# oss0430/SRFRD

Hardware: AMD Instinct MI355X
Metric: sequences/sec (higher is better)
Workload: dtype f32

## Files before the change

srfrd_amd/csrc/srfrd_encoder_bwd_ragged_kernel.inc:

```
namespace SRFRD_NS {


struct RagBwdLds {
  lds_f* base;
  lds_f* s_ln;
  lds_f* s_lng;
};

template <int K_, int DI_, bool RMW_, bool SEAM_ = false>
__device__ __forceinline__ void rag_bwd_seq(const EncArgs& a, const RagBwdLds& m, int b, int iter, int& tid, int wave, uint32_t seed,
                                            int seam_th = 0) {
  const Dims& ly = a.dm;
  constexpr int nw = 8, nthr = 512;
  constexpr int L = 50, D = 50, LP = 64, DK = 52, DS = 54, NT = 4, MT = 4;
  constexpr int R = 52, SZ = R * DS, SLD = R + 2, SH = kRagSH;
  static_assert(SH == LP - R && R * SLD <= SZ + 2 * R, "slot geometry");
  static_assert(kRagBwdWork == SH * DS + 6 * SZ + 13 * LP, "working set");
  constexpr bool CV2 = true;
  constexpr int CIT = (R * (D / 2) + nthr - 1) / nthr;
  constexpr int PIT = (R * (R / 2) + nthr - 1) / nthr;
  lds_f* slot[6];
#pragma unroll
  for (int s = 0; s < 6; ++s) slot[s] = m.base + SH * DS + s * SZ;
  lds_f* tail = m.base + SH * DS + 6 * SZ;
  lds_i* s_in = (lds_i*)tail;
  lds_f* s_keep = tail + LP;
  lds_i* s_pid = (lds_i*)(tail + 2 * LP);
  lds_i* s_nid = (lds_i*)(tail + 3 * LP);
  lds_i* s_fk = (lds_i*)(tail + 4 * LP);
  lds_i* s_pfk = (lds_i*)(tail + 5 * LP);
  lds_i* s_nfk = (lds_i*)(tail + 6 * LP);
  lds_f* s_dpl = tail + 7 * LP;
  lds_f* s_dnl = tail + 8 * LP;
  lds_f* s_delta = tail + 9 * LP;
  lds_f* s_brep = tail + 10 * LP;
  lds_f* s_dummy = tail + 11 * LP;
  lds_f* s_misc = tail + 12 * LP;
  lds_f* s_ln = m.s_ln;
  lds_f* s_lng = m.s_lng;
  const float* P = a.dense;
  const bool drop_on = a.drop_on != 0;
  const int rkind = K_ >= 0 ? K_ : ly.kind;
  const bool is_sas = rkind == SRFRD_SASREC;
  const bool has_fake = rkind == SRFRD_SRFR || rkind == SRFRD_SRFRN;
  const bool is_srfu = rkind >= SRFRD_SRFU_B;
  constexpr int di = DI_, dfk = D - DI_;
  constexpr int dout = (K_ == SRFRD_SRFR) ? DI_ : D;
  const float sqrtD = sqrtf((float)di);
  const float qscale = a.qscale;
  const int B = a.B;
  auto pk = [&](int mat, int form) {
    return PackedB{reinterpret_cast<const float4*>(a.packed) + ((int64_t)mat * 2 + form) * (kPackFloats / 4)};
  };
  static_assert(L <= nthr && (R - L) * DS <= nthr, "single-pass helpers");
  auto ones_col = [&](lds_f* buf) {
    if (tid < L) buf[tid * DS + D] = 1.0f;
  };
  auto zero_pad_rows = [&](lds_f* buf) {
    if (tid < (R - L) * DS) buf[L * DS + tid] = 0.f;
  };
  const float keep_scale = drop_on ? a.drop_scale : 1.0f;

  asm volatile("" : "+v"(tid));
  float* slab = a.grad_slabs + (int64_t)blockIdx.x * ly.n_dense;
  const int rmw = RMW_ ? (iter != 0) : 0;
  if (iter == 0)
    for (int i = tid; i < ly.blk0; i += nthr) slab[i] = 0.f;
  const int64_t rowbase = (int64_t)b * L;
  const uint32_t seq = (uint32_t)(a.seq0 + b);
  const int lane0 = tid & 63;
  if (tid < LP) {
    const int t = tid;
    const bool in = t < L;
    const int id = in ? clamp_id(a.in_ids[rowbase + t], ly.n_items) : 0;
    const int pid = (in && a.pos_ids) ? clamp_id(a.pos_ids[rowbase + t], ly.n_items) : 0;
    const int nid = (in && a.neg_ids) ? clamp_id(a.neg_ids[rowbase + t], ly.n_items) : 0;
    s_in[t] = id;
    s_keep[t] = id != 0 ? 1.f : 0.f;
    s_pid[t] = pid;
    s_nid[t] = nid;
    s_fk[t] = (in && a.fk_ids) ? clamp_id(a.fk_ids[rowbase + t], 2) : 0;
    s_pfk[t] = (in && a.pos_fk) ? clamp_id(a.pos_fk[rowbase + t], 2) : 0;
    s_nfk[t] = (in && a.neg_fk) ? clamp_id(a.neg_fk[rowbase + t], 2) : 0;
    float dp = 0.f, dn = 0.f;
    if constexpr (SEAM_) {
      if constexpr (K_ == SRFRD_SRFRN)
        if (in) {
          const float* dl = a.head_dh + (int64_t)B * L * dout + rowbase * 2;
          dp = dl[t];
          dn = dl[L + t];
        }
    } else if (in) {
      if (a.fused_bce) {
        const float pl = a.c_pl[rowbase + t], nl = a.c_nl[rowbase + t];
        bce_dlogits(pid, pl, nl, dp, dn);
      } else {
        if (a.d_pos && a.pos_ids) dp = a.d_pos[rowbase + t];
        if (a.d_neg && a.neg_ids) dn = a.d_neg[rowbase + t];
      }
    }
    s_dpl[t] = dp;
    s_dnl[t] = dn;
  }
  if (is_srfu && wave == 1) {
    const int lab = user_label_wave(rkind, a.fk_ids ? a.fk_ids + rowbase : nullptr, L, ly.n_labels);
    if (lane0 == 0) ((lds_i*)s_misc)[0] = lab;
  }
  __syncthreads();
  int t0, th;
  {
    const bool inr = lane0 < L;
    const unsigned long long nz = __ballot(inr && s_in[lane0] != 0);
    const unsigned long long ng = __ballot(inr && (s_in[lane0] != 0 || s_dpl[lane0] != 0.f || s_dnl[lane0] != 0.f));
    t0 = nz ? (int)__builtin_ctzll(nz) : L;
    th = ng ? (int)__builtin_ctzll(ng) : L;
    if (a.ragged_off) t0 = 0;
    if (a.d_hidden != nullptr || a.ragged_off) th = 0;
    if constexpr (SEAM_) th = seam_th;
    t0 = __builtin_amdgcn_readfirstlane(t0);
    th = __builtin_amdgcn_readfirstlane(th);
  }
  const int krp = t0 >= 1 ? t0 - 1 : 0;
  const int kr = krp + SH, v0 = t0 + SH;
  const int mt0 = kr >> 4, r0 = mt0 << 4, mtn = MT - mt0;
  const int p0 = r0 > SH ? r0 - SH : 0;
  const int k0 = p0 + SH;
  const RagHead hr = rag_head_range(th, krp);
  const int mh0 = hr.tile0, mhn = MT - mh0;
  const int ph0 = hr.pos0, kh0 = ph0 + SH;

  lds_f *sX = slot[0], *sQ = slot[1], *sG = slot[2], *sT = slot[3], *sK = slot[4], *sO = slot[5];
  lds_f* dummy = s_dummy;
#define TB(p) ((p) - SH * DS)
  G2L<CIT, CV2> g_last, g_h1, g_r;
  g_last.load(a.c_save_x + x_off(ly.n_blocks, b, ly.n_blocks, L, D) + p0 * D, L - p0, D, nthr);
  g_h1.load(a.c_save_h1 + h1_off(ly.n_blocks - 1, b, ly.n_blocks, L, D) + p0 * D, L - p0, D, nthr);
  g_r.load(a.c_save_aux + aux_off(ly.n_blocks - 1, b, ly.n_blocks, L, LP, D).r + p0 * D, L - p0, D, nthr);
  if constexpr (SEAM_) {
    constexpr bool V2 = dout % 2 == 0;
    constexpr int HIT = (L * (V2 ? dout / 2 : dout) + nthr - 1) / nthr;
    G2L<HIT, V2> g_dh;
    g_dh.load(a.head_dh + (rowbase + ph0) * dout, L - ph0, dout, nthr);
    g_dh.store(sG + ph0 * DS, DS, L - ph0, dout, nthr);
    if constexpr (K_ == SRFRD_SRFRN) {
      g_dh.load(a.c_hidden + (rowbase + ph0) * dout, L - ph0, dout, nthr);
      g_dh.store(sT + ph0 * DS, DS, L - ph0, dout, nthr);
    }
    if (dout < D)
      for (int idx = tid; idx < (L - ph0) * (D - dout); idx += nthr) {
        const int tt = idx / (D - dout), cc = dout + idx - tt * (D - dout);
        sG[(ph0 + tt) * DS + cc] = 0.f;
      }
  }
  g_last.store(sX + p0 * DS, DS, L - p0, D, nthr);
  for (int r = ph0 + (tid >> 6); r < p0; r += nthr >> 6) {
    const int c = tid & 63;
    if (c < DS && c != D) sX[r * DS + c] = 0.f;
  }
  zero_pad_rows(sX);
  ones_col(sX);
  zero_pad_rows(sG);
  __syncthreads();

  int lane = tid & 63, li = lane & 15, lq = lane >> 4;
#define RG_RELANE() do { asm volatile("" : "+v"(tid)); lane = tid & 63; li = lane & 15; lq = lane >> 4; } while (0)
  const int nt_w = wave & 3, g_w = wave >> 2;
  auto slab_gemm = [&](int kk0, auto amat, auto bmat, const SlabWB& sl, const SlabPre& pre) {
    f32x4 acc[2];
#pragma unroll
    for (int j = 0; j < 2; ++j) acc[j] = f32x4{pre.v[j][0], pre.v[j][1], pre.v[j][2], pre.v[j][3]};
    mma_group<2>(acc, amat, bmat, (g_w << 4) + li, 32, (nt_w << 4) + li, kk0, LP, lq);
    const SlabCol sc = slab_col(sl, (nt_w << 4) + li);
    if (sc.ok) {
#pragma unroll
      for (int j = 0; j < 2; ++j)
#pragma unroll
        for (int e = 0; e < 4; ++e) {
          const int r = ((g_w + 2 * j) << 4) + (lq << 2) + e;
          if (r < sl.R) sl.base[(unsigned)(sc.col0 + r * sc.rs)] = acc[j][e];
        }
    }
  };
  auto col_sums = [&](int kk0, const lds_f* m_b, lds_f* dst, int ncol) {
    if (wave < NT) {
      f32x4 acc[1] = {f32x4{0.f, 0.f, 0.f, 0.f}};
      mma_group<1>(acc, OnesRow{}, Mat{m_b, DS}, li, 0, (wave << 4) + li, kk0, LP, lq);
      const int c = (wave << 4) + li;
      if (lq == 0 && c < ncol) dst[c] += acc[0][0];
    }
  };
  auto side_sums = [&](int n_out, auto term, auto dst_off, int tlo) {
    for (int p = wave; p < n_out; p += nw) {
      float sacc = 0.f;
      for (int t = tlo + lane; t < L; t += 64) sacc += term(p, t);
      sacc = wave_sum(sacc);
      if (lane == 0) atomicAdd(&slab[dst_off(p)], sacc);
    }
  };

  const lds_f* lnin = sX;
  if (K_ == SRFRD_SRFR) {
    const WFrag wl = load_wfrag(pk(ly.n_blocks * 6, 0), P + ly.off_lc_b, di, (di + 15) >> 4, tid);
    {
      constexpr int nst = (di + 15) >> 4;
      const int nt3 = wave % nst, g3 = wave / nst;
      auto epi = [&](int r, int c, float v) { *((c < di && r >= SH && r < SH + L) ? &TB(sQ)[r * DS + c] : dummy + c) = v; };
      if (g3 < 2) {
        if (g3 + 2 < mhn) gemm_group_packed<2>(mh0 + g3, 2, nt3, DK >> 2, Mat{TB(sX), DS}, wl, epi, lane);
        else if (g3 < mhn) gemm_group_packed<1>(mh0 + g3, 2, nt3, DK >> 2, Mat{TB(sX), DS}, wl, epi, lane);
      }
    }
    __syncthreads();
    lnin = sQ;
  }
  if constexpr (!SEAM_) {
// ... 345 lines not shown
    col_sums(k0, TB(H), s_lng + (4 * i + 1) * 64, D);
    col_sums(k0, TB(GX1), s_lng + (4 * i + 0) * 64, D);
    __syncthreads();
    G = DX;
    fr[0] = H; fr[1] = GX1; fr[2] = Xb; fr[3] = N1; fr[4] = DQ;
  }

  RG_RELANE();
  {
    const DropSite dsE = drop_site(drop_on && is_sas, seed, SITE_EMB, seq, a.drop_thr, a.drop_scale);
    {
      int t = p0 + tid / di, c = tid - (tid / di) * di;
      constexpr int dt = nthr / di, dc = nthr - dt * di;
      for (; t < L;) {
        float gv = G[t * DS + c] * s_keep[t];
        if (is_sas) gv *= drop_mul(dsE, t, c);
        const int id = s_in[t];
        if (a.contrib != nullptr) a.contrib[(((int64_t)2 * B + b) * L + t) * di + c] = id != 0 ? (is_sas ? gv * sqrtD : gv) : 0.f;
        else if (id != 0) atomicAdd(&a.grad_table[(int64_t)id * di + c], is_sas ? gv * sqrtD : gv);
        atomicAdd(&slab[ly.off_pos + t * di + c], gv);
        t += dt; c += dc;
        if (c >= di) { c -= di; ++t; }
      }
      if (a.contrib != nullptr)
        for (int idx = tid; idx < p0 * di; idx += nthr) a.contrib[(((int64_t)2 * B + b) * L) * di + idx] = 0.f;
    }
    if (has_fake)
      side_sums(2 * dfk, [&](int p, int t) {
        constexpr int dq = dfk > 0 ? dfk : 1;
        const int f = 1 + p / dq, c = p - (f - 1) * dq;
        return s_fk[t] == f ? G[t * DS + di + c] * s_keep[t] : 0.f;
      }, [&](int p) { return ly.off_side + dfk + p; }, p0);
    if (is_srfu) {
      const int lab = ((lds_i*)s_misc)[0];
      side_sums(D, [&](int c, int t) { return G[t * DS + c] * s_keep[t]; }, [&](int c) { return ly.off_side + lab * D + c; }, p0);
    }
  }
  __syncthreads();
  for (int idx = tid; idx < (4 * ly.n_blocks + 2) * 64; idx += nthr) {
    const int vec = idx >> 6, c = idx & 63;
    if (vec < 4 * ly.n_blocks) {
      const BlkOff o = blk_off(ly.blk0 + (vec >> 2) * ly.blk_stride, D);
      const int sel = vec & 3;
      if (c < D) slab[(sel == 0 ? o.ln1_w : sel == 1 ? o.ln1_b : sel == 2 ? o.ln2_w : o.ln2_b) + c] = s_lng[idx];
    } else if (c < dout) {
      slab[(vec == 4 * ly.n_blocks ? ly.off_ll_w : ly.off_ll_b) + c] = s_lng[idx];
    }
  }
  __syncthreads();
#undef TB
#undef RG_RELANE
}

template <int K_, int DI_, bool RMW_>
__global__ void __launch_bounds__(512, 4) encoder_bwd_ragged_kernel(const EncArgs a) {
  extern __shared__ __attribute__((aligned(16))) float smem[];
  const Dims& ly = a.dm;
  constexpr int nthr = 512;
  int tid = threadIdx.x;
  const int wave = __builtin_amdgcn_readfirstlane(tid >> 6);
  const RagT0 t0v = rag_load_t0(a, tid);
  lds_f* base = (lds_f*)smem;
  {
    const int total = (int)bwd_ragged_lds_floats(ly.n_blocks);
    for (int i = tid; i < total; i += nthr) base[i] = 0.f;
  }
  lds_f* s_ln = base + kRagBwdWork;
  const RagBwdLds m{base, s_ln, s_ln + ln_cache_floats(ly.n_blocks)};
  __syncthreads();
  fill_ln_cache(s_ln, a.dense, ly);
  const uint32_t seed = a.seed_dev ? *a.seed_dev : a.seed;
  __syncthreads();

  STAMP_INIT
  for (int iter = 0;; ++iter) {
    const int b = __builtin_amdgcn_readfirstlane(rag_take(a, (lds_i*)(base + kRagSH * 54), iter, tid, t0v));
    if (b < 0) break;
    rag_bwd_seq<K_, DI_, RMW_>(a, m, b, iter, tid, wave, seed);
  }
}

}
```

srfrd_amd/csrc/srfrd_encoder_fwd_ragged_kernel.inc:

```
namespace SRFRD_NS {

constexpr int kRagSH = 12;

constexpr int kRagChunks = 2;
struct RagT0 {
  int v[kRagChunks];
};
__device__ __forceinline__ bool rag_ordered(const EncArgs& a) { return a.sched != nullptr && a.sched_mode != 0 && a.B <= 512 * kRagChunks; }
__device__ __forceinline__ RagT0 rag_load_t0(const EncArgs& a, int tid) {
  RagT0 t;
#pragma unroll
  for (int c = 0; c < kRagChunks; ++c) {
    const int b = c * 512 + tid;
    t.v[c] = (rag_ordered(a) && c * 512 < a.B) ? a.sched[kSchedT0 + min(b, a.B - 1)] : 0;
  }
  return t;
}

__device__ __forceinline__ int rag_select(const RagT0& t0v, int B, int want, lds_i* scr, int tid) {
  lds_i* hist = scr;
  lds_i* wcnt = scr + 64;
  lds_i* res = scr + 80;
  const int lane = tid & 63, wave = tid >> 6;
  constexpr int NCH = kRagChunks;
// ... 25 lines not shown
  int seen = 0;
#pragma unroll
  for (int c = 0; c < NCH; ++c) {
    if (c * 512 >= B) break;
    const int b = c * 512 + tid;
    const bool f = b < B && min(max(tv[c], 0), 63) == k;
    const unsigned long long m = __ballot(f);
    if (lane == 0) wcnt[wave] = (int)__builtin_popcountll(m);
    __syncthreads();
    int before = seen, total = 0;
#pragma unroll
    for (int w = 0; w < 8; ++w) {
      const int cw = wcnt[w];
      if (w < wave) before += cw;
      total += cw;
    }
    const int mine = before + (int)__builtin_popcountll(m & ((1ull << lane) - 1ull));
    if (f && mine == r) res[2] = b;
    seen += total;
    __syncthreads();
  }
  return res[2];
}

__device__ __forceinline__ int rag_take(const EncArgs& a, lds_i* scr, int iter, int tid, const RagT0& t0v) {
  const int x = (int)blockIdx.x + iter * (int)gridDim.x;
  if (x >= a.B) return -1;
  if (!rag_ordered(a)) return x;
  const int G = a.sched[kSchedG];
  const int want = x < G ? x : (x < 2 * G ? a.B - 1 - (x - G) : x - G);
  return rag_select(t0v, a.B, want, scr, tid);
}

__device__ __forceinline__ float softplus_fast(float z) { return fmaxf(z, 0.f) + __logf(1.0f + __expf(-fabsf(z))); }

__device__ __forceinline__ void bce_dlogits(int pid, float pl, float nl, float& dp, float& dn) {
  if (pid != 0) {
    dp = sigmoid_f(pl) - 1.0f;
    dn = sigmoid_f(nl);
  }
}
__device__ __forceinline__ float head_dh(float up, float dp, float pv, float dn, float nv) {
  up += dp * pv + dn * nv;
  return up;
}
template <int K_>
__device__ __forceinline__ float head_dh_as_backward(float dp, float pv, float dn, float nv) {
  float a = dp * pv;
  asm volatile("" : "+v"(a));
  if constexpr (K_ == SRFRD_SRFRN) return __builtin_fmaf(dn, nv, a);
  float b = dn * nv;
  asm volatile("" : "+v"(b));
  return a + b;
}
__device__ __forceinline__ float head_contrib(float dl, float h) { return dl * h; }
struct RagHead {
  int tile0, pos0;
};
__device__ __forceinline__ RagHead rag_head_range(int th, int krp) {
  const int hp = th < krp ? th : krp;
  RagHead r;
  r.tile0 = (hp + kRagSH) >> 4;
  const int rh0 = r.tile0 << 4;
  r.pos0 = rh0 > kRagSH ? rh0 - kRagSH : 0;
  return r;
}

struct NoPost {
  __device__ __forceinline__ void operator()(int, int, const float (&)[4]) const {}
};
template <int G, bool TWO, class AL, class AL2, class PRE, class EPI, class POST = NoPost>
__device__ __forceinline__ void rgemm_packed(int mt, int mstride_tiles, int nt, int ksteps, int ncols, const AL& a, const WFrag& w,
                                             const AL2& a2, const WFrag& w2, const PRE& pre, const EPI& epi, int lane,
                                             const POST& post = POST{}) {
  const int li = lane & 15, lq = lane >> 4;
  const int c = (nt << 4) + li;
  float pv[G][4];
#pragma unroll
  for (int j = 0; j < G; ++j)
#pragma unroll
    for (int e = 0; e < 4; ++e) pv[j][e] = pre(((mt + j * mstride_tiles) << 4) + (lq << 2) + e, c);
  f32x4 acc[G];
#pragma unroll
  for (int j = 0; j < G; ++j) acc[j] = f32x4{0.f, 0.f, 0.f, 0.f};
  const int mrow = (mt << 4) + li, mstride = mstride_tiles << 4;
#pragma unroll
  for (int pass = 0; pass < (TWO ? 2 : 1); ++pass) {
    float av[4][G];
#pragma unroll
    for (int s = 0; s < 4; ++s)
      if (s < ksteps)
#pragma unroll
        for (int j = 0; j < G; ++j) av[s][j] = pass == 0 ? a(mrow + j * mstride, 4 * s + lq) : a2(mrow + j * mstride, 4 * s + lq);
#pragma unroll
    for (int kc = 0; kc < kPackKC; ++kc) {
      const int nst = ksteps - 4 * kc;
      if (nst > 0) {
        const int nnext = nst - 4;
        float an[4][G];
#pragma unroll
        for (int s = 0; s < 4; ++s)
          if (s < nnext)
#pragma unroll
            for (int j = 0; j < G; ++j)
              an[s][j] = pass == 0 ? a(mrow + j * mstride, ((kc + 1) << 4) + 4 * s + lq) : a2(mrow + j * mstride, ((kc + 1) << 4) + 4 * s + lq);
        __builtin_amdgcn_sched_barrier(0);
// ... 139 lines not shown
    for (int i = 0; i < 4; ++i) { const f32x2 t = row2[i < npair ? i : 0]; x[2 * i] = t.x; x[2 * i + 1] = t.y; }
  }
  float mx = -INFINITY;
#pragma unroll
  for (int i = 0; i < 8; ++i) {
    const int pj = m8 + i;
    x[i] = (own && pj >= krp && pj <= ip) ? x[i] : -INFINITY;
    mx = fmaxf(mx, x[i]);
  }
  mx = row_max(mx);
  float s = 0.f;
#pragma unroll
  for (int i = 0; i < 8; ++i) {
    const int pj = m8 + i;
    const float e = (own && pj >= krp && pj <= ip) ? __expf(x[i] - mx) : 0.f;
    x[i] = e;
    s += (rep && pj == krp) ? e * (float)t0 : e;
  }
  s = row_sum(s);
  const float inv = 1.0f / s;
  float cnt = (float)t0;
  if (ds.on && rep) {
    int c = 0;
    for (int jj = tid & 7; jj < t0; jj += 8) c += drop_mul(ds, ip, jj) != 0.f ? 1 : 0;
    cnt = row_sum((float)c);
  }
  if (!own) return;
  const float scale = ds.on ? ds.scale : 1.0f;
  float pv[8], gs[8];
#pragma unroll
  for (int i = 0; i < 8; ++i) {
    const int pj = m8 + i;
    const float p = x[i] * inv;
    if (rep && pj == krp) {
      const float pm = p * cnt;
      if (gsave != nullptr) gsave[ip * LP + LP - 1] = p * (float)t0;
      pv[i] = pm * scale;
      gs[i] = pm;
    } else {
      const float mul = drop_mul(ds, ip, pj);
      pv[i] = p * mul;
      gs[i] = mul != 0.f ? p : -p;
    }
  }
#pragma unroll
  for (int i = 0; i < 4; ++i)
    if (i < npair) row2[i] = f32x2{pv[2 * i], pv[2 * i + 1]};
  if (g4 != nullptr) {
    g4[0] = make_float4(gs[0], gs[1], gs[2], gs[3]);
    g4[1] = make_float4(gs[4], gs[5], gs[6], gs[7]);
  }
}

struct RagFwdLds {
  lds_f *bXS, *bQN, *bQ, *bK, *bV;
  lds_i* s_in;
  lds_f* s_keep;
  lds_i *s_pid, *s_nid;
  lds_f* s_misc;
  lds_f* s_ln;
};

template <int K_, int T_, int DI_, bool SEAM_ = false>
__device__ __forceinline__ int rag_fwd_seq(const EncArgs& a, const RagFwdLds& m, int b, int& tid, int wave, uint32_t seed) {
  static_assert(!SEAM_ || T_ != 0, "the head seam belongs to the training forward");
  const Dims& ly = a.dm;
  constexpr int D = 50, L = 50, LP = 64, DK = 52, DS = 54, SLD = 66, NT = 4, MT = 4, SH = kRagSH;
  constexpr int nw = 8, nthr = 512;
  static_assert(SH + L <= LP && (SH & 3) == 0, "tile coordinates");
  const int lane0 = threadIdx.x & 63;
  lds_f* bXS = m.bXS;
  lds_f* bQN = m.bQN;
  lds_f* bQ = m.bQ;
  lds_f* bK = m.bK;
  lds_f* bV = m.bV;
  lds_i* s_in = m.s_in;
  lds_f* s_keep = m.s_keep;
  lds_i* s_pid = m.s_pid;
  lds_i* s_nid = m.s_nid;
  lds_f* s_misc = m.s_misc;
  lds_f* s_ln = m.s_ln;
  const float* P = a.dense;
  const ItemTable table{a.table, a.table16};
  constexpr bool TR_ = T_ != 0;
  const bool has_pos = TR_ || a.pos_ids != nullptr, has_neg = TR_ || a.neg_ids != nullptr;
  const bool drop_on = TR_ || a.drop_on != 0, do_save = TR_ || a.save_x != nullptr, do_loss = TR_ || a.loss_part != nullptr;
  const int kind = K_ >= 0 ? K_ : ly.kind;
  const bool is_sas = kind == SRFRD_SASREC;
  const bool has_fake = kind == SRFRD_SRFR || kind == SRFRD_SRFRN;
  const bool is_srfu = kind >= SRFRD_SRFU_B;
  constexpr int di = DI_, dfk = D - DI_;
  constexpr int dout = (K_ == SRFRD_SRFR) ? DI_ : D;
  const float sqrtD = sqrtf((float)di);
  const float qscale = a.qscale;
  auto pk = [&](int mat, int form) {
    return PackedB{reinterpret_cast<const float4*>(a.packed) + ((int64_t)mat * 2 + form) * (kPackFloats / 4)};
  };

  asm volatile("" : "+v"(tid));
  const int64_t rowbase = (int64_t)b * L;
  const uint32_t seq = (uint32_t)(a.seq0 + b);
  if (tid < LP) {
    const int t = tid - SH;
    const bool in = t >= 0 && t < L;
    const int id = in ? clamp_id(a.in_ids[rowbase + t], ly.n_items) : 0;
    s_in[tid] = id;
    s_keep[tid] = id != 0 ? 1.f : 0.f;
    s_pid[tid] = (in && has_pos) ? clamp_id(a.pos_ids[rowbase + t], ly.n_items) : 0;
    s_nid[tid] = (in && has_neg) ? clamp_id(a.neg_ids[rowbase + t], ly.n_items) : 0;
  }
  if (is_srfu && wave == 1) {
    const int lab = user_label_wave(kind, a.fk_ids ? a.fk_ids + rowbase : nullptr, L, ly.n_labels);
    if (lane0 == 0) ((lds_i*)s_misc)[0] = lab;
  }
  __syncthreads();
  int v0;
  {
// ... 108 lines not shown
        const int r = r_ + rq0;
        if (c < D) {
          bQ[r * DS + c] = v;
          if (sv_o && (unsigned)(r - SH) < (unsigned)L) sv_o[(unsigned)((r - SH) * D + c)] = v;
        }
      };
      if (lo) {
        if (g == 0) {
          const int kk0 = r0 > SH ? r0 : SH;
          gemm_group<0, 1>(0, 1, nt << 4, LP - kk0, Mat{bXS + rq0 * SLD + kk0, SLD}, Mat{bV + kk0 * DS, DS}, epi_o, li, lq);
        }
      } else {
        const int kk0 = r0 > SH ? r0 : SH;
        const Mat Ap{bXS + r0 * SLD + kk0, SLD};
        const Mat Bv{bV + kk0 * DS, DS};
        const int kend = LP - kk0;
        int ma, mb;
        if (mtn == 4) { ma = g == 0 ? 0 : 1; mb = g == 0 ? 3 : 2; }
        else if (mtn == 3) { ma = g == 0 ? 2 : 0; mb = g == 0 ? -1 : 1; }
        else if (mtn == 2) { ma = g == 0 ? 1 : 0; mb = -1; }
        else { ma = g == 0 ? 0 : -1; mb = -1; }
        if (ma >= 0) gemm_group<2, 1>(ma, 1, nt << 4, kend, Ap, Bv, epi_o, li, lq);
        if (mb >= 0) gemm_group<2, 1>(mb, 1, nt << 4, kend, Ap, Bv, epi_o, li, lq);
      }
    }
    __syncthreads();
    rag_packed(mq0, mqn, DK >> 2, D, Mat{bQ, DS}, wo, [&](int r, int c) { return bQN[r * DS + c]; }, [&](int r, int c, float v, float res) {
      const float h = res + v;
      bXS[r * DS + c] = h;
      return h;
    }, lane, wave, [&](int rb, int c, const float (&gv)[4]) { if (do_save) gstore4(a.save_h1 + h1_off(i, b, ly.n_blocks, L, D), rb, c, gv); });
    __syncthreads();
    ln_rows(nw, bXS + rq0 * DS, bQN + rq0 * DS, LP - rq0, DS, D, s_ln + (4 * i + 2) * 64, s_ln + (4 * i + 3) * 64);
    __syncthreads();
    const DropSite ds1 = drop_site(drop_on, seed, site_ffn1(i), seq, a.drop_thr, a.drop_scale);
    const DropSite ds2 = drop_site(drop_on, seed, site_ffn2(i), seq, a.drop_thr, a.drop_scale);
    const WFrag w2 = load_wfrag(pk(i * 6 + 5, 0), P + o.c2_b, D, NT, tid);
    rag_packed(mq0, mqn, DK >> 2, D, Mat{bQN, DS}, w1, NoPre{}, [&](int r, int c, float v, float) {
      const float h = fmaxf(v * drop_mul(ds1, r - SH, c), 0.f);
      bQ[r * DS + c] = h;
      return h;
    }, lane, wave, [&](int rb, int c, const float (&gv)[4]) { if (sv_r) gstore4(sv_r, rb, c, gv); });
    __syncthreads();
    rag_packed(mq0, mqn, DK >> 2, D, Mat{bQ, DS}, w2, [&](int r, int c) { return bQN[r * DS + c]; }, [&](int r, int c, float v, float res) {
      const float y = (v * drop_mul(ds2, r - SH, c) + res) * s_keep[r];
      bXS[r * DS + c] = y;
      return y;
    }, lane, wave, [&](int rb, int c, const float (&gv)[4]) { if (do_save) gstore4(a.save_x + x_off(i + 1, b, ly.n_blocks, L, D), rb, c, gv); });
    __syncthreads();
  }

  const bool lo_h = !TR_ && a.last_only != 0;
  int seam_th = 0;
  asm volatile("" : "+v"(tid));
  const int lane = tid & 63;
  if (!lo_h && r0 > SH) {
    for (int i = tid; i < (r0 - SH) * DS; i += nthr) bXS[SH * DS + i] = 0.f;
    __syncthreads();
  }
  lds_f* xp = bXS + SH * DS;
  lds_f* qnp = bQN + SH * DS;
  const lds_f* hin = xp;
  const int p0h = lo_h ? L - 1 : 0;
  if (kind == SRFRD_SRFR) {
    const WFrag wl = load_wfrag(pk(ly.n_blocks * 6, 0), P + ly.off_lc_b, di, (di + 15) >> 4, tid);
    const int mh0 = lo_h ? MT - 1 : 0;
    {
      constexpr int nst = (di + 15) >> 4;
      const int nt = wave % nst, g = wave / nst;
      const int mtn_h = MT - mh0;
      auto epi = [&](int r_, int c, float v) { if (c < di) bQ[(r_ + (mh0 << 4)) * DS + c] = v; };
      if (g < 2) {
        if (g + 2 < mtn_h) gemm_group_packed<2>(g, 2, nt, DK >> 2, Mat{bXS + (mh0 << 4) * DS, DS}, wl, epi, lane);
        else if (g < mtn_h) gemm_group_packed<1>(g, 2, nt, DK >> 2, Mat{bXS + (mh0 << 4) * DS, DS}, wl, epi, lane);
      }
    }
    __syncthreads();
    hin = bQ + SH * DS;
  }
  ln_rows(nw, hin + p0h * DS, qnp + p0h * DS, L - p0h, DS, dout, s_ln + (4 * ly.n_blocks) * 64, s_ln + (4 * ly.n_blocks + 1) * 64);
  __syncthreads();
  if (lo_h) {
    for (int c = tid; c < dout; c += nthr) a.hidden[(int64_t)b * dout + c] = qnp[(L - 1) * DS + c];
  } else {
    const bool srfrn = kind == SRFRD_SRFRN;
    lds_f* kp = bK + SH * DS;
    lds_f* vp = bV + SH * DS;
    lds_f* s_dp = bXS + LP * DS;
    lds_f* s_dn = s_dp + LP;
    static_assert(LP * DS + 2 * LP <= LP * SLD, "logit gradients inside the x / scores matrix");
    {
      int t = tid / dout, c = tid - t * dout;
      constexpr int dt = nthr / dout, dc = nthr - dt * dout;
      for (; t < L;) {
        const float h = qnp[t * DS + c];
        a.hidden[(rowbase + t) * dout + c] = h;
        if (has_pos) {
          const float pv = c < di ? table((int64_t)s_pid[t + SH] * di + c)
                                  : (srfrn ? P[ly.off_side + clamp_id(a.pos_fk[rowbase + t], 2) * dfk + (c - di)] : 0.f);
          kp[t * DS + c] = h * pv;
          if constexpr (SEAM_) xp[t * DS + c] = pv;
        }
        if (has_neg) {
          const float nv = c < di ? table((int64_t)s_nid[t + SH] * di + c)
                                  : (srfrn ? P[ly.off_side + clamp_id(a.neg_fk[rowbase + t], 2) * dfk + (c - di)] : 0.f);
          vp[t * DS + c] = h * nv;
          if constexpr (SEAM_) bQ[(t + SH) * DS + c] = nv;
        }
        t += dt; c += dc;
        if (c >= dout) { c -= dout; ++t; }
      }
    }
    __syncthreads();
    float sp = 0.f, sn = 0.f, cnt = 0.f;
    const int q = tid & (kRL - 1);
    for (int t = tid / kRL; t < L; t += nthr / kRL) {
      float ap = 0.f, an = 0.f;
#pragma unroll
      for (int j = 0; j < kQC; ++j) {
        const int c = q + kRL * j;
        if (c < dout) {
          if (has_pos) ap += kp[t * DS + c];
          if (has_neg) an += vp[t * DS + c];
        }
      }
      const float pl = row_sum(ap), nl = row_sum(an);
      if (q == 0) {
        if (has_pos) a.pos_logits[rowbase + t] = pl;
        if (has_neg) a.neg_logits[rowbase + t] = nl;
        if constexpr (SEAM_) {
          float dp = 0.f, dn = 0.f;
          bce_dlogits(s_pid[t + SH], pl, nl, dp, dn);
          s_dp[t] = dp;
          s_dn[t] = dn;
        }
        if (do_loss && s_pid[t + SH] != 0) {
          sp += softplus_fast(-pl);
          sn += softplus_fast(nl);
          cnt += 1.f;
        }
      }
    }
    if (do_loss) {
      sp = wave_sum(sp); sn = wave_sum(sn); cnt = wave_sum(cnt);
      if (lane == 0) {
        s_misc[8 + wave * 3 + 0] = sp;
        s_misc[8 + wave * 3 + 1] = sn;
        s_misc[8 + wave * 3 + 2] = cnt;
      }
      __syncthreads();
      if (tid < 3) {
        float s = 0.f;
        for (int w = 0; w < nw; ++w) s += s_misc[8 + w * 3 + tid];
        a.loss_part[(int64_t)b * 3 + tid] = s;
      }
    }
    if constexpr (SEAM_) {
      const int l0 = tid & 63;
      const unsigned long long ng = __ballot(l0 < L && (s_in[l0 + SH] != 0 || s_dp[l0] != 0.f || s_dn[l0] != 0.f));
      seam_th = ng ? (int)__builtin_ctzll(ng) : L;
      if (a.ragged_off) seam_th = 0;
      seam_th = __builtin_amdgcn_readfirstlane(seam_th);
      const int ph0 = rag_head_range(seam_th, t0 >= 1 ? t0 - 1 : 0).pos0;
      float* dhb = a.head_dh + (rowbase + ph0) * dout;
      const int B = a.B;
      int t = ph0 + tid / dout, c = tid - (tid / dout) * dout, i = tid;
      constexpr int dt = nthr / dout, dc = nthr - dt * dout;
      for (; t < L;) {
        const float dp = s_dp[t], dn = s_dn[t];
        float dh = 0.f;
        if (c < di || srfrn) dh = head_dh_as_backward<K_>(dp, xp[t * DS + c], dn, bQ[(t + SH) * DS + c]);
        dhb[i] = dh;
        if (c < di) {
          const float h = qnp[t * DS + c];
          const int pid = s_pid[t + SH], nid = s_nid[t + SH];
          if (a.contrib != nullptr) {
            a.contrib[(((int64_t)0 * B + b) * L + t) * di + c] = pid != 0 ? head_contrib(dp, h) : 0.f;
            a.contrib[(((int64_t)1 * B + b) * L + t) * di + c] = nid != 0 ? head_contrib(dn, h) : 0.f;
          } else {
            if (pid != 0 && dp != 0.f) atomicAdd(&a.grad_table[(int64_t)pid * di + c], head_contrib(dp, h));
            if (nid != 0 && dn != 0.f) atomicAdd(&a.grad_table[(int64_t)nid * di + c], head_contrib(dn, h));
          }
        }
        t += dt; c += dc; i += nthr;
        if (c >= dout) { c -= dout; ++t; }
      }
      if (a.contrib != nullptr)
        for (int idx = tid; idx < ph0 * di; idx += nthr) {
          a.contrib[(((int64_t)0 * B + b) * L) * di + idx] = 0.f;
          a.contrib[(((int64_t)1 * B + b) * L) * di + idx] = 0.f;
        }
      if constexpr (K_ == SRFRD_SRFRN)
        if (tid < L) {
          float* dl = a.head_dh + (int64_t)B * L * dout + rowbase * 2;
          dl[tid] = s_dp[tid];
          dl[L + tid] = s_dn[tid];
        }
    }
  }
  __syncthreads();
  return seam_th;
}

template <int K_, int T_, int DI_>
__global__ void __launch_bounds__(512, 4) encoder_fwd_ragged_kernel(const EncArgs a) {
  extern __shared__ __attribute__((aligned(16))) float smem[];
  const Dims& ly = a.dm;
  constexpr int D = 50, L = 50, LP = 64, DS = 54, SLD = 66;
  constexpr int nthr = 512;
  int tid = threadIdx.x;
  const int wave = __builtin_amdgcn_readfirstlane(tid >> 6);
  constexpr int szA = LP * DS, szX = LP * SLD;
  const int tailsz = 4 * LP + 64 + ln_cache_floats(ly.n_blocks);
  const RagT0 t0v = rag_load_t0(a, tid);
  lds_f* c_cur = (lds_f*)smem;
  auto carve = [&](int64_t n) -> lds_f* { lds_f* p = c_cur; c_cur += n; return p; };
  {
    Geom g = make_geom(L, D);
    const int total = (int)fwd_lds_floats(g, ly.n_blocks);
    for (int i = tid; i < total; i += nthr) ((lds_f*)smem)[i] = 0.f;
  }
  lds_f* tail = carve(tailsz);
  RagFwdLds m;
  m.bXS = carve(szX);
  m.bQN = carve(szA);
  m.bQ = carve(szA);
  m.bK = carve(szA);
  m.bV = carve(szA + kSlack);
  m.s_in = (lds_i*)tail;
  m.s_keep = tail + LP;
  m.s_pid = (lds_i*)(tail + 2 * LP);
  m.s_nid = (lds_i*)(tail + 3 * LP);
  m.s_misc = tail + 4 * LP;
  lds_f* s_ln = m.s_misc + 64;
  m.s_ln = s_ln;
  __syncthreads();
  fill_ln_cache(s_ln, a.dense, ly);
  const uint32_t seed = a.seed_dev ? *a.seed_dev : a.seed;

  STAMP_INIT
  for (int iter = 0;; ++iter) {
    const int b = __builtin_amdgcn_readfirstlane(rag_take(a, (lds_i*)m.bXS, iter, tid, t0v));
    if (b < 0) break;
    rag_fwd_seq<K_, T_, DI_>(a, m, b, tid, wave, seed);
  }
}

}
```

srfrd_amd/csrc/srfrd_encoder_train_ragged.hip:

```cpp
#include "srfrd_enc_common.h"

#include "srfrd_encoder_fwd_ragged_kernel.inc"
#include "srfrd_encoder_bwd_ragged_kernel.inc"

namespace srfrd {

template <int K_, int DI_, bool RMW_>
__global__ void __launch_bounds__(512, 4) encoder_train_ragged_kernel(const EncArgs a) {
  extern __shared__ __attribute__((aligned(16))) float smem[];
  const Dims& ly = a.dm;
  constexpr int LP = 64, DS = 54, SLD = 66, nthr = 512;
  constexpr int W = kRagFwdWork > kRagBwdWork ? kRagFwdWork : kRagBwdWork;
  int tid = threadIdx.x;
  const int wave = __builtin_amdgcn_readfirstlane(tid >> 6);
  const RagT0 t0v = rag_load_t0(a, tid);
  lds_f* base = (lds_f*)smem;
  {
    const int total = (int)train_ragged_lds_floats(ly.n_blocks);
    for (int i = tid; i < total; i += nthr) base[i] = 0.f;
  }
  RagFwdLds fm;
  fm.bXS = base;
  fm.bQN = base + LP * SLD;
  fm.bQ = fm.bQN + LP * DS;
  fm.bK = fm.bQ + LP * DS;
  fm.bV = fm.bK + LP * DS;
  lds_f* ftail = fm.bV + LP * DS;
  fm.s_in = (lds_i*)ftail;
  fm.s_keep = ftail + LP;
  fm.s_pid = (lds_i*)(ftail + 2 * LP);
  fm.s_nid = (lds_i*)(ftail + 3 * LP);
  fm.s_misc = ftail + 4 * LP;
  static_assert(LP * SLD + 4 * LP * DS + 5 * LP == kRagFwdWork, "forward working set");
  lds_f* s_ln = base + W;
  fm.s_ln = s_ln;
  const RagBwdLds bm{base, s_ln, s_ln + ln_cache_floats(ly.n_blocks)};
  __syncthreads();
  fill_ln_cache(s_ln, a.dense, ly);
  const uint32_t seed = a.seed_dev ? *a.seed_dev : a.seed;

  for (int iter = 0;; ++iter) {
    if (iter > 0) {
      for (int i = tid; i < W; i += nthr) base[i] = 0.f;
      __syncthreads();
    }
    const int b = __builtin_amdgcn_readfirstlane(rag_take(a, (lds_i*)fm.bXS, iter, tid, t0v));
    if (b < 0) break;
    const int th = rag_fwd_seq<K_, 1, DI_, true>(a, fm, b, tid, wave, seed);
    for (int i = tid; i < W; i += nthr) base[i] = 0.f;
    __syncthreads();
    rag_bwd_seq<K_, DI_, RMW_, true>(a, bm, b, iter, tid, wave, seed, th);
  }
}

int launch_train_ragged(const KernelPlan& k, const EncArgs& a, void* stream) {
  return with_variant(k.variant, [&](auto v) {
    constexpr KindVariant kv = kKindVariants[decltype(v)::value];
    return with_flag(k.flag, [&](auto rmw) { return launch_enc(encoder_train_ragged_kernel<kv.K, kv.DI, decltype(rmw)::value>, k, stream, a); });
  });
}

}

using namespace srfrd;

extern "C" int64_t srfrd_train_scratch_floats(const srfrd_layout* lay, int B, int L) {
  if (!lay || B <= 0 || L <= 0) return 0;
  return (int64_t)B * L * (lay->d_out + (lay->kind == SRFRD_SRFRN ? 2 : 0));
}

extern "C" int srfrd_encoder_train_sched(const srfrd_layout* lay, const void* item_table, const float* dense, const float* packed,
                                         const int64_t* input_ids, const int64_t* fake_ids, const int64_t* pos_ids,
                                         const int64_t* pos_fake, const int64_t* neg_ids, const int64_t* neg_fake, int B, int L,
                                         double dropout_p, uint32_t seed, const uint32_t* seed_dev, int64_t seq_index0,
                                         float* hidden, float* pos_logits, float* neg_logits, float* save_x, float* save_h1,
                                         float* save_aux, float* loss_part, const float* d_hidden, const float* d_pos,
                                         const float* d_neg, int fused_bce, float* grad_table, float* table_contrib,
                                         float* grad_slabs, float* scratch, int64_t scratch_floats, const int32_t* sched,
                                         int sched_mode, void* stream) {
  if (sched_mode < 0 || sched_mode > 1 || (sched_mode != 0 && !sched)) return SRFRD_E_ARG;
  const int sw = read_switches();
  EncArgs a = {};
  a.sched = sched_mode != 0 ? sched : nullptr;
  a.sched_mode = a.sched ? sched_mode : 0;
  a.ragged_off = (sw & SRFRD_SW_RAGGED_FULL_ROWS) != 0;
  const int rc = fill_args(a, lay, item_table, dense, packed, input_ids, fake_ids, pos_ids, pos_fake, neg_ids, neg_fake, B, L,
                           dropout_p, seed, seed_dev, seq_index0);
  if (rc) return rc;
  if (!hidden || (pos_ids && !pos_logits) || (neg_ids && !neg_logits)) return SRFRD_E_ARG;
  if (loss_part && !(pos_ids && neg_ids)) return SRFRD_E_ARG;
  if ((save_x != nullptr) != (save_h1 != nullptr) || (save_x != nullptr) != (save_aux != nullptr)) return SRFRD_E_ARG;
  if (!save_x || !grad_table || !grad_slabs) return SRFRD_E_ARG;
  if (fused_bce && !(pos_ids && neg_ids)) return SRFRD_E_ARG;
  const int mode = (pos_ids ? SRFRD_PLAN_POS : 0) | (neg_ids ? SRFRD_PLAN_NEG : 0) | SRFRD_PLAN_CKPT | (loss_part ? SRFRD_PLAN_LOSS : 0) |
                   (dropout_p > 0.0 ? SRFRD_PLAN_DROPOUT : 0) | (fused_bce && !d_hidden ? SRFRD_PLAN_FUSED_BCE : 0);
  const KernelPlan k = encoder_plan(*lay, B, L, mode, sw, num_cu(), scratch ? scratch_floats : 0).train;
  if (k.rc) return k.rc;
  if (!scratch || scratch_floats < srfrd_train_scratch_floats(lay, B, L)) return SRFRD_E_ARG;
  a.head_dh = scratch;
  a.hidden = hidden; a.pos_logits = pos_logits; a.neg_logits = neg_logits;
  a.save_x = save_x; a.save_h1 = save_h1; a.save_aux = save_aux; a.loss_part = loss_part;
  a.c_hidden = hidden; a.c_pl = pos_logits; a.c_nl = neg_logits; a.c_save_x = save_x; a.c_save_h1 = save_h1; a.c_save_aux = save_aux;
  a.fused_bce = 1;
  a.grad_table = grad_table; a.grad_slabs = grad_slabs; a.contrib = table_contrib;
  return launch_train_ragged(k, a, stream);
}
```

Baseline: 3.060 million.

## Hand off head gradient and metadata through LDS instead of global scratch

In the fused train kernel, the forward head seam now writes d_hidden straight into the LDS slot the backward pass reads, rather than into a global scratch buffer that the backward then reloads. Per-token ids, fake ids and dlogits travel in registers through a RagSeam struct, and the final-layer activations already in LDS are reused instead of reloaded from save_x. The full LDS zeroing is replaced by selective zeroing that avoids the live regions. This removes global round trips and a barrier per sequence, at the cost of more fragile LDS aliasing between the forward and backward layouts.

Measured after the change: 3.121 million, median of 6. +2.0%, better.

```diff
diff --git a/srfrd_amd/csrc/srfrd_encoder_bwd_ragged_kernel.inc b/srfrd_amd/csrc/srfrd_encoder_bwd_ragged_kernel.inc
--- a/srfrd_amd/csrc/srfrd_encoder_bwd_ragged_kernel.inc
+++ b/srfrd_amd/csrc/srfrd_encoder_bwd_ragged_kernel.inc
@@ -9,7 +9,7 @@
 
 template <int K_, int DI_, bool RMW_, bool SEAM_ = false>
 __device__ __forceinline__ void rag_bwd_seq(const EncArgs& a, const RagBwdLds& m, int b, int iter, int& tid, int wave, uint32_t seed,
-                                            int seam_th = 0) {
+                                            const RagSeam& hs = RagSeam{}) {
   const Dims& ly = a.dm;
   constexpr int nw = 8, nthr = 512;
   constexpr int L = 50, D = 50, LP = 64, DK = 52, DS = 54, NT = 4, MT = 4;
@@ -69,7 +69,7 @@
   const int64_t rowbase = (int64_t)b * L;
   const uint32_t seq = (uint32_t)(a.seq0 + b);
   const int lane0 = tid & 63;
-  if (tid < LP) {
+  if (!SEAM_ && tid < LP) {
     const int t = tid;
     const bool in = t < L;
     const int id = in ? clamp_id(a.in_ids[rowbase + t], ly.n_items) : 0;
@@ -83,14 +83,7 @@
     s_pfk[t] = (in && a.pos_fk) ? clamp_id(a.pos_fk[rowbase + t], 2) : 0;
     s_nfk[t] = (in && a.neg_fk) ? clamp_id(a.neg_fk[rowbase + t], 2) : 0;
     float dp = 0.f, dn = 0.f;
-    if constexpr (SEAM_) {
-      if constexpr (K_ == SRFRD_SRFRN)
-        if (in) {
-          const float* dl = a.head_dh + (int64_t)B * L * dout + rowbase * 2;
-          dp = dl[t];
-          dn = dl[L + t];
-        }
-    } else if (in) {
+    if (in) {
       if (a.fused_bce) {
         const float pl = a.c_pl[rowbase + t], nl = a.c_nl[rowbase + t];
         bce_dlogits(pid, pl, nl, dp, dn);
@@ -106,9 +99,12 @@
     const int lab = user_label_wave(rkind, a.fk_ids ? a.fk_ids + rowbase : nullptr, L, ly.n_labels);
     if (lane0 == 0) ((lds_i*)s_misc)[0] = lab;
   }
-  __syncthreads();
+  if constexpr (!SEAM_) __syncthreads();
   int t0, th;
-  {
+  if constexpr (SEAM_) {
+    t0 = hs.t0;
+    th = hs.th;
+  } else {
     const bool inr = lane0 < L;
     const unsigned long long nz = __ballot(inr && s_in[lane0] != 0);
     const unsigned long long ng = __ballot(inr && (s_in[lane0] != 0 || s_dpl[lane0] != 0.f || s_dnl[lane0] != 0.f));
@@ -116,7 +112,6 @@
     th = ng ? (int)__builtin_ctzll(ng) : L;
     if (a.ragged_off) t0 = 0;
     if (a.d_hidden != nullptr || a.ragged_off) th = 0;
-    if constexpr (SEAM_) th = seam_th;
     t0 = __builtin_amdgcn_readfirstlane(t0);
     th = __builtin_amdgcn_readfirstlane(th);
   }
@@ -129,38 +124,34 @@
   const int mh0 = hr.tile0, mhn = MT - mh0;
   const int ph0 = hr.pos0, kh0 = ph0 + SH;
 
-  lds_f *sX = slot[0], *sQ = slot[1], *sG = slot[2], *sT = slot[3], *sK = slot[4], *sO = slot[5];
+  static_assert(kRagSlot == SZ && kRagSeamG == 3, "hand-off slot");
+  lds_f *sX = slot[0], *sQ = slot[1], *sG = slot[SEAM_ ? 3 : 2], *sT = slot[SEAM_ ? 2 : 3], *sK = slot[4], *sO = slot[5];
   lds_f* dummy = s_dummy;
 #define TB(p) ((p) - SH * DS)
   G2L<CIT, CV2> g_last, g_h1, g_r;
-  g_last.load(a.c_save_x + x_off(ly.n_blocks, b, ly.n_blocks, L, D) + p0 * D, L - p0, D, nthr);
+  if constexpr (!SEAM_) g_last.load(a.c_save_x + x_off(ly.n_blocks, b, ly.n_blocks, L, D) + p0 * D, L - p0, D, nthr);
   g_h1.load(a.c_save_h1 + h1_off(ly.n_blocks - 1, b, ly.n_blocks, L, D) + p0 * D, L - p0, D, nthr);
   g_r.load(a.c_save_aux + aux_off(ly.n_blocks - 1, b, ly.n_blocks, L, LP, D).r + p0 * D, L - p0, D, nthr);
   if constexpr (SEAM_) {
-    constexpr bool V2 = dout % 2 == 0;
-    constexpr int HIT = (L * (V2 ? dout / 2 : dout) + nthr - 1) / nthr;
-    G2L<HIT, V2> g_dh;
-    g_dh.load(a.head_dh + (rowbase + ph0) * dout, L - ph0, dout, nthr);
-    g_dh.store(sG + ph0 * DS, DS, L - ph0, dout, nthr);
     if constexpr (K_ == SRFRD_SRFRN) {
-      g_dh.load(a.c_hidden + (rowbase + ph0) * dout, L - ph0, dout, nthr);
-      g_dh.store(sT + ph0 * DS, DS, L - ph0, dout, nthr);
-    }
-    if (dout < D)
-      for (int idx = tid; idx < (L - ph0) * (D - dout); idx += nthr) {
-        const int tt = idx / (D - dout), cc = dout + idx - tt * (D - dout);
-        sG[(ph0 + tt) * DS + cc] = 0.f;
-      }
-  }
-  g_last.store(sX + p0 * DS, DS, L - p0, D, nthr);
-  for (int r = ph0 + (tid >> 6); r < p0; r += nthr >> 6) {
-    const int c = tid & 63;
-    if (c < DS && c != D) sX[r * DS + c] = 0.f;
-  }
-  zero_pad_rows(sX);
-  ones_col(sX);
-  zero_pad_rows(sG);
-  __syncthreads();
+      constexpr bool V2 = dout % 2 == 0;
+      constexpr int HIT = (L * (V2 ? dout / 2 : dout) + nthr - 1) / nthr;
+      G2L<HIT, V2> g_hid;
+      g_hid.load(a.c_hidden + (rowbase + ph0) * dout, L - ph0, dout, nthr);
+      g_hid.store(sT + ph0 * DS, DS, L - ph0, dout, nthr);
+      __syncthreads();
+    }
+  } else {
+    g_last.store(sX + p0 * DS, DS, L - p0, D, nthr);
+    for (int r = ph0 + (tid >> 6); r < p0; r += nthr >> 6) {
+      const int c = tid & 63;
+      if (c < DS && c != D) sX[r * DS + c] = 0.f;
+    }
+    zero_pad_rows(sX);
+    ones_col(sX);
+    zero_pad_rows(sG);
+    __syncthreads();
+  }
 
   int lane = tid & 63, li = lane & 15, lq = lane >> 4;
 #define RG_RELANE() do { asm volatile("" : "+v"(tid)); lane = tid & 63; li = lane & 15; lq = lane >> 4; } while (0)
@@ -612,6 +603,46 @@
 #undef RG_RELANE
 }
 
+template <int K_, int DI_>
+__device__ __forceinline__ void rag_seam_handoff(const RagBwdLds& m, const RagSeam& hs, int W, int tid) {
+  constexpr int nthr = 512, L = 50, D = 50, LP = 64, DS = 54, R = 52, SZ = R * DS, SH = kRagSH;
+  constexpr int dout = (K_ == SRFRD_SRFR) ? DI_ : D;
+  constexpr int oX = SH * DS, oG = oX + kRagSeamG * SZ, oT = oX + 6 * SZ, nT = 9 * LP;
+  lds_f* base = m.base;
+  const int krp = hs.t0 >= 1 ? hs.t0 - 1 : 0;
+  const int r0 = ((krp + SH) >> 4) << 4;
+  const int p0 = r0 > SH ? r0 - SH : 0;
+  const int ph0 = rag_head_range(hs.th, krp).pos0;
+  auto zero = [&](int lo, int hi) {
+    for (int i = lo + tid; i < hi; i += nthr) base[i] = 0.f;
+  };
+  zero(0, oX);
+  zero(oX + SZ, oG);
+  zero(oG + SZ, oT);
+  zero(oT + nT, W);
+  {
+    const int c = tid & 63;
+    if (c < DS)
+      for (int r = tid >> 6; r < R; r += nthr >> 6) {
+        if (!(r >= p0 && r < L && c < D)) base[oX + r * DS + c] = (c == D && r < L) ? 1.0f : 0.f;
+        if (!(r >= ph0 && r < L && c < dout)) base[oG + r * DS + c] = 0.f;
+      }
+  }
+  if (tid < LP) {
+    lds_f* tail = base + oT;
+    lds_i* ti = (lds_i*)tail;
+    ti[tid] = hs.id;
+    tail[LP + tid] = hs.id != 0 ? 1.f : 0.f;
+    ti[2 * LP + tid] = hs.pid;
+    ti[3 * LP + tid] = hs.nid;
+    ti[4 * LP + tid] = hs.fk;
+    ti[5 * LP + tid] = hs.pfk;
+    ti[6 * LP + tid] = hs.nfk;
+    tail[7 * LP + tid] = hs.dp;
+    tail[8 * LP + tid] = hs.dn;
+  }
+}
+
 template <int K_, int DI_, bool RMW_>
 __global__ void __launch_bounds__(512, 4) encoder_bwd_ragged_kernel(const EncArgs a) {
   extern __shared__ __attribute__((aligned(16))) float smem[];
diff --git a/srfrd_amd/csrc/srfrd_encoder_fwd_ragged_kernel.inc b/srfrd_amd/csrc/srfrd_encoder_fwd_ragged_kernel.inc
--- a/srfrd_amd/csrc/srfrd_encoder_fwd_ragged_kernel.inc
+++ b/srfrd_amd/csrc/srfrd_encoder_fwd_ragged_kernel.inc
@@ -101,6 +101,11 @@
   float b = dn * nv;
   asm volatile("" : "+v"(b));
   return a + b;
+}
+__device__ __forceinline__ float seam_product(float h, float v) {
+  float p = h * v;
+  asm volatile("" : "+v"(p));
+  return p;
 }
 __device__ __forceinline__ float head_contrib(float dl, float h) { return dl * h; }
 struct RagHead {
@@ -346,6 +351,14 @@
   }
 }
 
+struct RagSeam {
+  int th, t0;
+  int id, pid, nid, fk, pfk, nfk;
+  float dp, dn;
+};
+constexpr int kRagSlot = 52 * 54;
+constexpr int kRagSeamG = 3;
+
 struct RagFwdLds {
   lds_f *bXS, *bQN, *bQ, *bK, *bV;
   lds_i* s_in;
@@ -356,7 +369,7 @@
 };
 
 template <int K_, int T_, int DI_, bool SEAM_ = false>
-__device__ __forceinline__ int rag_fwd_seq(const EncArgs& a, const RagFwdLds& m, int b, int& tid, int wave, uint32_t seed) {
+__device__ __forceinline__ RagSeam rag_fwd_seq(const EncArgs& a, const RagFwdLds& m, int b, int& tid, int wave, uint32_t seed) {
   static_assert(!SEAM_ || T_ != 0, "the head seam belongs to the training forward");
   const Dims& ly = a.dm;
   constexpr int D = 50, L = 50, LP = 64, DK = 52, DS = 54, SLD = 66, NT = 4, MT = 4, SH = kRagSH;
@@ -571,6 +584,7 @@
 
   const bool lo_h = !TR_ && a.last_only != 0;
   int seam_th = 0;
+  RagSeam hs = {};
   asm volatile("" : "+v"(tid));
   const int lane = tid & 63;
   if (!lo_h && r0 > SH) {
@@ -617,14 +631,12 @@
         if (has_pos) {
           const float pv = c < di ? table((int64_t)s_pid[t + SH] * di + c)
                                   : (srfrn ? P[ly.off_side + clamp_id(a.pos_fk[rowbase + t], 2) * dfk + (c - di)] : 0.f);
-          kp[t * DS + c] = h * pv;
-          if constexpr (SEAM_) xp[t * DS + c] = pv;
+          kp[t * DS + c] = SEAM_ ? pv : h * pv;
         }
         if (has_neg) {
           const float nv = c < di ? table((int64_t)s_nid[t + SH] * di + c)
                                   : (srfrn ? P[ly.off_side + clamp_id(a.neg_fk[rowbase + t], 2) * dfk + (c - di)] : 0.f);
-          vp[t * DS + c] = h * nv;
-          if constexpr (SEAM_) bQ[(t + SH) * DS + c] = nv;
+          vp[t * DS + c] = SEAM_ ? nv : h * nv;
         }
         t += dt; c += dc;
         if (c >= dout) { c -= dout; ++t; }
@@ -639,8 +651,14 @@
       for (int j = 0; j < kQC; ++j) {
         const int c = q + kRL * j;
         if (c < dout) {
-          if (has_pos) ap += kp[t * DS + c];
-          if (has_neg) an += vp[t * DS + c];
+          if constexpr (SEAM_) {
+            const float h = qnp[t * DS + c];
+            ap += seam_product(h, kp[t * DS + c]);
+            an += seam_product(h, vp[t * DS + c]);
+          } else {
+            if (has_pos) ap += kp[t * DS + c];
+            if (has_neg) an += vp[t * DS + c];
+          }
         }
       }
       const float pl = row_sum(ap), nl = row_sum(an);
@@ -681,15 +699,22 @@
       if (a.ragged_off) seam_th = 0;
       seam_th = __builtin_amdgcn_readfirstlane(seam_th);
       const int ph0 = rag_head_range(seam_th, t0 >= 1 ? t0 - 1 : 0).pos0;
-      float* dhb = a.head_dh + (rowbase + ph0) * dout;
+      hs.th = seam_th;
+      hs.t0 = t0;
+      if (has_fake && tid < L) {
+        hs.fk = a.fk_ids ? clamp_id(a.fk_ids[rowbase + tid], 2) : 0;
+        hs.pfk = a.pos_fk ? clamp_id(a.pos_fk[rowbase + tid], 2) : 0;
+        hs.nfk = a.neg_fk ? clamp_id(a.neg_fk[rowbase + tid], 2) : 0;
+      }
+      lds_f* sgp = xp + kRagSeamG * kRagSlot;
       const int B = a.B;
-      int t = ph0 + tid / dout, c = tid - (tid / dout) * dout, i = tid;
+      int t = ph0 + tid / dout, c = tid - (tid / dout) * dout;
       constexpr int dt = nthr / dout, dc = nthr - dt * dout;
       for (; t < L;) {
         const float dp = s_dp[t], dn = s_dn[t];
         float dh = 0.f;
-        if (c < di || srfrn) dh = head_dh_as_backward<K_>(dp, xp[t * DS + c], dn, bQ[(t + SH) * DS + c]);
-        dhb[i] = dh;
+        if (c < di || srfrn) dh = head_dh_as_backward<K_>(dp, kp[t * DS + c], dn, vp[t * DS + c]);
+        sgp[t * DS + c] = dh;
         if (c < di) {
           const float h = qnp[t * DS + c];
           const int pid = s_pid[t + SH], nid = s_nid[t + SH];
@@ -701,7 +726,7 @@
             if (nid != 0 && dn != 0.f) atomicAdd(&a.grad_table[(int64_t)nid * di + c], head_contrib(dn, h));
           }
         }
-        t += dt; c += dc; i += nthr;
+        t += dt; c += dc;
         if (c >= dout) { c -= dout; ++t; }
       }
       if (a.contrib != nullptr)
@@ -709,16 +734,19 @@
           a.contrib[(((int64_t)0 * B + b) * L) * di + idx] = 0.f;
           a.contrib[(((int64_t)1 * B + b) * L) * di + idx] = 0.f;
         }
-      if constexpr (K_ == SRFRD_SRFRN)
-        if (tid < L) {
-          float* dl = a.head_dh + (int64_t)B * L * dout + rowbase * 2;
-          dl[tid] = s_dp[tid];
-          dl[L + tid] = s_dn[tid];
-        }
+      if (tid < L) {
+        hs.id = s_in[tid + SH];
+        hs.pid = s_pid[tid + SH];
+        hs.nid = s_nid[tid + SH];
+        if constexpr (K_ == SRFRD_SRFRN) {
+          hs.dp = s_dp[tid];
+          hs.dn = s_dn[tid];
+        }
+      }
     }
   }
   __syncthreads();
-  return seam_th;
+  return hs;
 }
 
 template <int K_, int T_, int DI_>
diff --git a/srfrd_amd/csrc/srfrd_encoder_train_ragged.hip b/srfrd_amd/csrc/srfrd_encoder_train_ragged.hip
--- a/srfrd_amd/csrc/srfrd_encoder_train_ragged.hip
+++ b/srfrd_amd/csrc/srfrd_encoder_train_ragged.hip
@@ -32,6 +32,8 @@
   fm.s_nid = (lds_i*)(ftail + 3 * LP);
   fm.s_misc = ftail + 4 * LP;
   static_assert(LP * SLD + 4 * LP * DS + 5 * LP == kRagFwdWork, "forward working set");
+  constexpr int oG = (kRagSH + kRagSeamG * 52) * DS;
+  static_assert(oG >= LP * SLD + LP * DS && oG + 50 * DS <= LP * SLD + 2 * LP * DS + kRagSH * DS, "d hidden lands in dead floats");
   lds_f* s_ln = base + W;
   fm.s_ln = s_ln;
   const RagBwdLds bm{base, s_ln, s_ln + ln_cache_floats(ly.n_blocks)};
@@ -46,10 +48,10 @@
     }
     const int b = __builtin_amdgcn_readfirstlane(rag_take(a, (lds_i*)fm.bXS, iter, tid, t0v));
     if (b < 0) break;
-    const int th = rag_fwd_seq<K_, 1, DI_, true>(a, fm, b, tid, wave, seed);
-    for (int i = tid; i < W; i += nthr) base[i] = 0.f;
+    const RagSeam hs = rag_fwd_seq<K_, 1, DI_, true>(a, fm, b, tid, wave, seed);
+    rag_seam_handoff<K_, DI_>(bm, hs, W, tid);
     __syncthreads();
-    rag_bwd_seq<K_, DI_, RMW_, true>(a, bm, b, iter, tid, wave, seed, th);
+    rag_bwd_seq<K_, DI_, RMW_, true>(a, bm, b, iter, tid, wave, seed, hs);
   }
 }
 
@@ -97,7 +99,6 @@
   const KernelPlan k = encoder_plan(*lay, B, L, mode, sw, num_cu(), scratch ? scratch_floats : 0).train;
   if (k.rc) return k.rc;
   if (!scratch || scratch_floats < srfrd_train_scratch_floats(lay, B, L)) return SRFRD_E_ARG;
-  a.head_dh = scratch;
   a.hidden = hidden; a.pos_logits = pos_logits; a.neg_logits = neg_logits;
   a.save_x = save_x; a.save_h1 = save_h1; a.save_aux = save_aux; a.loss_part = loss_part;
   a.c_hidden = hidden; a.c_pl = pos_logits; a.c_nl = neg_logits; a.c_save_x = save_x; a.c_save_h1 = save_h1; a.c_save_aux = save_aux;
```
